# GreenleafLab/NucleoATAC

Measured on AMD Instinct MI355X. Metric: Mbp/s through occ+nuc signal pipeline, higher is better.
Workload: dtype f64

## Files before the change

### nucleoatac_amd/csrc/natac_api.hip

```cpp
#include "../../include/natac.h"
#ifndef NATAC_GNBL
#define NATAC_GNBL 2
#endif
#include "natac_kernels.hpp"
#include "natac_fft_bg.hpp"
#include "natac_occ_fast.hpp"
#include "natac_cand.hpp"
#include "natac_covsweep.hpp"
#include "natac_textz.hpp"
#include "natac_cores.hpp"
#include "natac_writer.hpp"
#include "natac_tabix.hpp"
#include "natac_pack.hpp"
#include "natac_bam.hpp"
#include "natac_bam_dev.hpp"
#include "natac_fragfile.hpp"
#include "natac_fragfile_dev.hpp"
#include "natac_fasta.hpp"
#include "natac_fuzzfit.hpp"
#include "natac_bedtab.hpp"
#include "natac_runtime.hpp"
#include "natac_pwmfit.hpp"
#include "natac_sites.hpp"
#include "natac_cellcounts.hpp"
#include "natac_cellqc.hpp"
#include "natac_peakcall.hpp"
#include "natac_tracks.hpp"
#include "natac_dropins.hpp"
#include "natac_trackio.hpp"
#include "natac_files.hpp"
#include "natac_store.hpp"
#include "natac_profile.hpp"

#include <algorithm>
#include <cmath>
#include <cstdio>
#include <cstring>
#include <limits>
#include <string>
#include <vector>

using namespace natac;

static int need_nuc_geometry(const natac_batch *b, const char *who) {
    const natac_ctx *c = b->ctx;
    const BatchOutputs &o = b->out;
    if (o.nuc_w < 0 || (o.nuc_w == c->vw && o.nuc_lower == c->vlower && o.nuc_upper == c->vupper)) return NATAC_OK;
    return fail(NATAC_E_STATE, "%s: natac_run_nuc ran with the V-plot geometry lower=%d upper=%d w=%d, the context now holds lower=%d "
                "upper=%d w=%d: run natac_run_nuc again", who, o.nuc_lower, o.nuc_upper, o.nuc_w, c->vlower, c->vupper, c->vw);
}
static int need_occ_geometry(const natac_batch *b, const char *who) {
    const natac_ctx *c = b->ctx;
    const BatchOutputs &o = b->out;
    if (o.occ_step < 0 || (o.occ_step == c->step && o.occ_half == c->halfstep && o.occ_flank == c->flank && o.occ_upper == c->occ_upper))
        return NATAC_OK;
    return fail(NATAC_E_STATE, "%s: natac_run_occ ran with step=%d flank=%d upper=%d, the context now holds step=%d flank=%d upper=%d: "
                "run natac_run_occ again", who, o.occ_step, o.occ_flank, o.occ_upper, c->step, c->flank, c->occ_upper);
}

static int choose_bg_G(const natac_batch *b, int W) {
    const int cand[4] = {7, 9, 13, 17};
    double best = 1e300;
    int bestG = 9;
    const int stride = std::max(1, b->nc / 65536);
    for (int ci = 0; ci < 4; ++ci) {
        const int G = cand[ci], TW = 64 * G;
        double cost = 0;
        for (int i = 0; i < b->nc; i += stride) {
            const int nt = (b->h_len[i] + TW - 1) / TW;
            cost += (double)nt * (TW + (W - 1) * 0.15 * 8);
        }
        if (cost < best) { best = cost; bestG = G; }
    }
    return bestG;
}

static void launch_candidates(natac_ctx *c, const ChunkTable &ct, const VMatDev &vm, const int *d_cc, const int *d_cp, long long n,
                              const double *nuc_cov, const double *norm, const double *bnum, const double *bcov, double *lr,
                              double *var, double *z, const long long *tile_first = nullptr, const int2 *ranges256 = nullptr) {
    const int EW = c->W + ((c->vupper - 2) >> 1) + ((c->vupper - 1) >> 1);
    const int ZN = (((c->vupper - 2) >> 1) + ((c->vupper - 1) >> 1) + 5 + 32) & ~1, ON = (c->W + 1) & ~1;
    const size_t lds4 = ((size_t)4 * CAND_PER_WAVE * ((EW + 1) & ~1) + ZN + ON) * sizeof(double);
    const bool per_wave = c->W <= 2 * WAVE;
    const size_t ldsp = (size_t)4 * CAND_PER_WAVE * CANDP_STRIDE * sizeof(double);
    bool paired = per_wave && bnum && bcov && c->vlower >= 2 && (c->R & 1) == 0 && c->W >= 64 && !vm.has_zero && EW <= CANDP_STRIDE &&
                  !getenv("NATAC_CAND_FULL") && !getenv("NATAC_CAND_OLD");
    if (paired && (c->lrt_gen != c->model_gen || !c->d_lrt)) {
        if (c->d_lrt.size() < (size_t)c->R * c->W && dev_alloc(c->d_lrt, (size_t)c->R * c->W) != NATAC_OK)
            paired = false;
        if (paired) {
            hipLaunchKernelGGL(natac_lr_table, dim3((unsigned)((c->R * c->W + 255) / 256)), dim3(256), 0, c->stream, c->d_vmat, c->d_srow, c->R, c->W,
                               c->d_lrt);
            c->lrt_gen = c->model_gen;
        }
    }
    if (paired) {
        VMatDev vml = vm;
        vml.lrt = c->d_lrt;
        const long long per_block = 4 * CAND_PER_WAVE;
        const dim3 grid((unsigned)((n + per_block - 1) / per_block));
        if (c->vlower & 1)
            hipLaunchKernelGGL((natac_candidates_paired<true>), grid, dim3(256), ldsp, c->stream, ct, vml, d_cc, d_cp, (int)n, nuc_cov, norm,
                               bnum, bcov, tile_first, ranges256, lr, var, z);
        else
            hipLaunchKernelGGL((natac_candidates_paired<false>), grid, dim3(256), ldsp, c->stream, ct, vml, d_cc, d_cp, (int)n, nuc_cov, norm,
                               bnum, bcov, tile_first, ranges256, lr, var, z);
        return;
    }
    if (per_wave && lds4 <= 64 * 1024) {
        const long long per_block = 4 * CAND_PER_WAVE;
        if (bnum && bcov && !getenv("NATAC_CAND_FULL"))
            hipLaunchKernelGGL((natac_candidates4<true>), dim3((unsigned)((n + per_block - 1) / per_block)), dim3(256), lds4, c->stream,
                               ct, vm, d_cc, d_cp, (int)n, nuc_cov, norm, bnum, bcov, lr, var, z);
        else
            hipLaunchKernelGGL((natac_candidates4<false>), dim3((unsigned)((n + per_block - 1) / per_block)), dim3(256), lds4, c->stream,
                               ct, vm, d_cc, d_cp, (int)n, nuc_cov, norm, bnum, bcov, lr, var, z);
    } else {
        hipLaunchKernelGGL(natac_candidates, dim3((unsigned)n), dim3(256), (size_t)(EW + 2) * sizeof(double), c->stream, ct, vm, d_cc,
                           d_cp, nuc_cov, norm, lr, var, z);
    }
}

template <int G>
static void launch_bg(natac_batch *b, const ChunkTable &ct, const VMatDev &vm) {
    natac_ctx *c = b->ctx;
    constexpr int W = 121;
    const int PW = 64 * G + W - 1;
    const int EW = PW + ((vm.upper - 2) >> 1) + ((vm.upper - 1) >> 1);
    const size_t lds = ((size_t)((EW + 1) & ~1) + PW) * sizeof(double);
    hipLaunchKernelGGL((natac_background<G, W>), dim3(b->n_tiles_bg), dim3(64), lds, c->stream, ct, b->d_tiles_bg, vm,
                       b->d_track[NATAC_T_NUC_COV], b->d_track[NATAC_T_RAW], b->d_track[NATAC_T_BACKGROUND],
                       b->d_track[NATAC_T_NORM], b->d_bnum, b->d_bcov);
}

struct OccFastLaunch { natac_batch *b; const ChunkTable &ct; const OccFastDev &of; size_t lds_gs, lds_od; int rem; bool rn16; };
template <int STEP, int REM = 0>
static void occ_gsum_launch(const OccFastLaunch &f) {
    if constexpr (REM < STEP) {
        if (f.rem == REM)
            hipLaunchKernelGGL((natac_occ_gsum<STEP, REM>), dim3(f.b->n_tiles_gs), dim3(256), f.lds_gs, f.b->ctx->stream, f.ct, f.b->d_tiles_gs, f.of,
                               f.b->d_blk_off, f.b->total_blocks, f.b->d_gsum);
        else
            occ_gsum_launch<STEP, REM + 1>(f);
    }
}
template <int STEP>
static void occ_fast_launch(const OccFastLaunch &f) {
    natac_batch *b = f.b;
    occ_gsum_launch<STEP>(f);
    auto kd = (f.of.flags & 2) ? (f.rn16 ? natac_occ_decide<STEP, 16, true> : natac_occ_decide<STEP, 4, true>)
                               : (f.rn16 ? natac_occ_decide<STEP, 16, false> : natac_occ_decide<STEP, 4, false>);
    const bool heavy_first = b->ctx->occ_ordered;
    hipLaunchKernelGGL(kd, dim3((b->n_tiles_occ + (heavy_first ? HEAVY_CAP : 0) + 3) / 4), dim3(256), f.lds_od, b->ctx->stream, f.ct, b->d_tiles_occ,
                       b->n_tiles_occ, b->d_ranges_occ, heavy_first ? b->d_order_occ : nullptr, f.of, b->d_blk_off, b->total_blocks, b->d_gsum, b->d_grid[0], b->d_grid[1], b->d_grid[2], b->d_defer,
                       b->d_defer + 1);
}

extern "C" {

int natac_abi_version(void) { return NATAC_ABI_VERSION; }
const char *natac_last_error(void) { return g_err.c_str(); }

int natac_device_count(int *count) {
    if (!count) return fail(NATAC_E_ARG, "count is NULL");
    int n = 0;
    hipError_t e = hipGetDeviceCount(&n);
    if (e != hipSuccess) {
        *count = 0;
        return fail(NATAC_E_HIP, "hipGetDeviceCount: %s", hipGetErrorString(e));
    }
    *count = n;
    return NATAC_OK;
}

int natac_ctx_create(int device_id, natac_ctx **out) {
    if (!out) return fail(NATAC_E_ARG, "out is NULL");
    *out = nullptr;
    int n = 0;
    HIPCHK(hipGetDeviceCount(&n));
    if (device_id < 0 || device_id >= n) return fail(NATAC_E_ARG, "device %d out of range (%d devices)", device_id, n);
    HIPCHK(hipSetDevice(device_id));
// ... 274 lines not shown
    if (rc) return rc;
    HIPCHK(sync_all(b->ctx));
    return NATAC_OK;
}

static int ensure_fft(natac_ctx *c) {
    int rc;
    if (!c->d_fft_tw) {
        std::vector<double> tw(2 * (size_t)natac::FFT_N);
        for (int k = 0; k < natac::FFT_N; ++k) {
            const double a = 2.0 * M_PI * k / natac::FFT_N;
            tw[2 * k] = std::cos(a);
            tw[2 * k + 1] = -std::sin(a);
        }
        if (const char *e = getenv("NATAC_FAULT_TWIDDLE")) {
            int k = 0; double dlt = 0.0;
            if (sscanf(e, "%d:%lf", &k, &dlt) == 2 && k >= 0 && k < natac::FFT_N) tw[2 * (size_t)k] += dlt;
        }
        if ((rc = dev_upload(c, c->d_fft_tw, tw.data(), tw.size()))) return rc;
        HIPCHK(sync_all(c));
    }
    if (!c->fft_dirty) return NATAC_OK;
    HIPCHK(sync_all(c));
    const int npair = (c->R + 1) / 2;
    if ((rc = dev_alloc(c->d_fft_k, (size_t)npair * 2 * natac::FFT_N))) return rc;
    hipLaunchKernelGGL(natac_fft_template, dim3(npair), dim3(64), 0, c->stream, c->d_vmat, c->d_srow, c->R, c->W, c->d_fft_tw, c->d_fft_k);
    if (c->W >= natac::FFT_EXT) {
        c->d_fft_mtab.reset(); c->d_fft_swt.reset();
        const int NJ = (c->R + 3) / 4;
        if ((rc = dev_alloc(c->d_fft_mtab, (size_t)2 * NJ * 64)) || (rc = dev_alloc(c->d_fft_swt, (size_t)4 * NJ))) return rc;
        hipLaunchKernelGGL(natac_fft_edge_table_mfma, dim3((2 * NJ * 64 + 255) / 256), dim3(256), 0, c->stream, c->d_vmat, c->d_srow, c->R, c->W, NJ,
                           c->d_fft_mtab, c->d_fft_swt);
    }
    HIPCHK(hipGetLastError());
    c->fft_dirty = false;
    return NATAC_OK;
}

static int ensure_window(natac_ctx *c, PoolBuf<double> &slot, int *slotM, double *slotsd, int M, double sd, double *slotsum = nullptr) {
    if (slot && *slotM == M && *slotsd == sd) return NATAC_OK;
    HIPCHK(sync_all(c));
    std::vector<double> w((size_t)M);
    for (int i = 0; i < M; ++i) {
        double n = (double)i - (M - 1) / 2.0;
        double q = n / sd;
        w[i] = std::exp(-0.5 * (q * q));
    }
    int rc = dev_upload(c, slot, w.data(), (size_t)M);
    if (rc) return rc;
    HIPCHK(sync_all(c));
    if (slotsum) {
        double acc = 0.0;
        for (int i = 0; i < M; ++i) acc = acc + w[i];
        *slotsum = acc;
    }
    *slotM = M;
    *slotsd = sd;
    return NATAC_OK;
}

static int run_exp_bias(natac_batch *b, hipStream_t st, bool from_occ) {
    if (!b->d_bias) return NATAC_OK;
    if (from_occ && b->ebias_fresh) { b->ebias_fresh = false; return NATAC_OK; }
    b->ebias_fresh = !from_occ;
    int rc;
    if (!b->d_ebias && (rc = dev_alloc(b->d_ebias, (size_t)b->nb))) return rc;
    const int blocks = (int)std::min<long long>((b->nb + 255) / 256, 16384);
    hipLaunchKernelGGL(natac_exp_bias, dim3(blocks), dim3(256), 0, st, b->d_bias, b->d_ebias, b->nb);
    return NATAC_OK;
}

static ChunkTable make_table(natac_batch *b) {
    ChunkTable t;
    t.nc = b->nc; t.chunk_len = b->d_len; t.frag_off = b->d_frag_off; t.lpos = b->d_lpos; t.ilen = b->d_ilen;
    t.centre = b->d_centre; t.bias_off = b->d_bias_off; t.bias = b->d_bias; t.ebias = b->d_ebias; t.bias_left = b->bias_left;
    t.bias_right = b->bias_right; t.out_off = b->d_out_off; t.grid_off = b->d_grid_off;
    return t;
}
static VMatDev make_vmat(natac_ctx *c) {
    VMatDev v;
    v.mat = c->d_vmat; v.matp = c->d_vmat_pad; v.srow = c->d_srow; v.lower = c->vlower; v.upper = c->vupper; v.w = c->vw; v.R = c->R; v.W = c->W;
    v.has_zero = (c->vmat_zero || c->srow_zero) ? 1 : 0;
    v.lrt = nullptr;
    return v;
}
static OccModelDev make_occ(natac_ctx *c) {
    OccModelDev o;
    o.nuc_probs = c->d_nucp; o.nfr_probs = c->d_nfrp; o.alphas = c->d_alphas; o.upper = c->occ_upper;
    o.n_alpha = c->n_alpha; o.step = c->step; o.halfstep = c->halfstep; o.flank = c->flank; o.cutoff = c->cutoff;
    o.ci_factor = std::exp(-0.5 * c->cutoff);
    o.zero_flags = c->occ_zero_flags;
    o.b_floor = c->occ_b_floor;
    return o;
}

static int build_tiles(natac_batch *b, int width, PoolBuf<int2> &d_out, int *n_out, bool grid_units = false, int step = 1, int half = 0) {
    std::vector<int2> tiles;
    tiles.reserve((size_t)(b->total_bp / std::max(1, width)) + b->nc);
    for (int i = 0; i < b->nc; ++i) {
        int n = b->h_len[i];
        if (grid_units) n = (b->h_len[i] > half) ? (b->h_len[i] - half + step - 1) / step : 0;
        for (int x = 0; x < n; x += width) tiles.push_back(make_int2(i, x));
    }
    *n_out = (int)tiles.size();
    int rc = dev_upload(b->ctx, d_out, tiles.data(), tiles.size());
    if (rc) return rc;
    HIPCHK(sync_all(b->ctx));
    return NATAC_OK;
}

int natac_batch_create(natac_ctx *c, int32_t nc, const int32_t *chunk_len, const int64_t *frag_off, const int32_t *frag_lpos,
                       const int32_t *frag_ilen, const int64_t *bias_off, const double *bias_log, int32_t bias_left,
                       int32_t bias_right, natac_batch **out) {
    if (!c || !out || !chunk_len || !frag_off) return fail(NATAC_E_ARG, "null argument");
    *out = nullptr;
    if (nc <= 0) return fail(NATAC_E_ARG, "n_chunks must be positive");
    if (bias_log && !bias_off) return fail(NATAC_E_ARG, "bias_log without bias_off");
    if (frag_off[0] != 0) return fail(NATAC_E_ARG, "frag_off[0] must be 0");
    const long long nf = frag_off[nc];
    if (nf > 0 && (!frag_lpos || !frag_ilen)) return fail(NATAC_E_ARG, "fragment arrays are NULL");
    HIPCHK(hipSetDevice(c->device));
    natac_batch *b = new natac_batch();
    b->ctx = c; b->nc = nc; b->nf = nf; b->bias_left = bias_left; b->bias_right = bias_right;
    b->h_len.assign(chunk_len, chunk_len + nc);
    b->h_out_off.resize((size_t)nc + 1);
    b->h_out_off[0] = 0;
    for (int i = 0; i < nc; ++i) {
        if (chunk_len[i] <= 0) { delete b; return fail(NATAC_E_ARG, "chunk %d has length %d", i, chunk_len[i]); }
        if (frag_off[i + 1] < frag_off[i] || frag_off[i + 1] - frag_off[i] > 0x7fffffffLL) {
            delete b; return fail(NATAC_E_ARG, "frag_off not monotone (chunk %d)", i);
        }
        if (bias_off && bias_off[i + 1] - bias_off[i] != (long long)chunk_len[i] + bias_left + bias_right) {
            delete b; return fail(NATAC_E_ARG, "bias slice of chunk %d must cover [start-%d, end+%d)", i, bias_left, bias_right);
        }
        b->h_out_off[i + 1] = b->h_out_off[i] + chunk_len[i];
    }
    b->total_bp = b->h_out_off[nc];
    b->nb = bias_off ? bias_off[nc] : 0;
    auto upload = [&]() -> int {
        int rc;
        if ((rc = dev_upload(c, b->d_len, chunk_len, (size_t)nc)) ||
            (rc = dev_upload(c, b->d_frag_off, (const long long *)frag_off, (size_t)nc + 1)) ||
            (rc = dev_upload(c, b->d_lpos, frag_lpos, (size_t)nf)) || (rc = dev_upload(c, b->d_ilen, frag_ilen, (size_t)nf)) ||
            (rc = dev_alloc(b->d_centre, (size_t)nf)) || (rc = dev_upload(c, b->d_out_off, b->h_out_off.data(), (size_t)nc + 1)))
            return rc;
        if (bias_off) {
            if ((rc = dev_upload(c, b->d_bias_off, (const long long *)bias_off, (size_t)nc + 1))) return rc;
            if (bias_log) rc = dev_upload(c, b->d_bias, bias_log, (size_t)b->nb);
            else rc = dev_alloc(b->d_bias, (size_t)b->nb);
            if (rc) return rc;
        }
        if ((rc = dev_alloc(b->d_status, (size_t)nc))) return rc;
        hipError_t e = hipMemsetAsync(b->d_status, 0, (size_t)nc * sizeof(int), c->stream);
        if (e != hipSuccess) return fail(NATAC_E_HIP, "memset: %s", hipGetErrorString(e));
        if (nf > 0) {
            int blocks = (int)std::min<long long>((nf + 255) / 256, 4096);
            hipLaunchKernelGGL(natac_frag_centres, dim3(blocks), dim3(256), 0, c->stream, b->d_lpos, b->d_ilen, b->d_centre, nf);
        }
        if ((rc = build_tiles(b, 256, b->d_tiles256, &b->n_tiles256))) return rc;
        {
            std::vector<long long> first((size_t)nc + 1, 0);
            for (int i = 0; i < nc; ++i) first[(size_t)i + 1] = first[i] + (chunk_len[i] + 255) / 256;
            if ((rc = dev_upload(c, b->d_tile256_first, first.data(), first.size()))) return rc;
        }
        e = hipStreamSynchronize(c->stream);
        if (e != hipSuccess) return fail(NATAC_E_HIP, "upload: %s", hipGetErrorString(e));
// ... 1046 lines not shown
```

### nucleoatac_amd/csrc/natac_cand.hpp

```cpp
#pragma once
#include "natac_kernels.hpp"

namespace natac {

__device__ __forceinline__ int row_lower_bound(const int *__restrict__ a, int lo, int hi, int key, int l, int sh) {
    while (__ballot(hi - lo > 16) != 0ull) {
        const int n = hi - lo;
        const bool big = n > 16;
        const int stride = big ? (n + 15) / 16 : 1;
        const int pi = min((l + 1) * stride - 1, max(n - 1, 0));
        const bool less = big && a[lo + pi] < key;
        const int cnt = __popc((unsigned)(__ballot(less) >> sh) & 0xffffu);
        if (big) {
            lo = min(lo + cnt * stride, hi);
            hi = min(lo + stride, hi);
        }
    }
    const int i = lo + l;
    const bool less = (i < hi) && a[i] < key;
    return lo + __popc((unsigned)(__ballot(less) >> sh) & 0xffffu);
}

__global__ void __launch_bounds__(256) natac_lr_table(const double *__restrict__ vmat, const double *__restrict__ srow, int R, int W,
                                                        double *__restrict__ out) {
    const int i = blockIdx.x * 256 + threadIdx.x;
    if (i < R * W) out[i] = log(vmat[i] / srow[i / W]);
}

constexpr int CANDP_STRIDE = 376;

template <bool LODD>
__global__ void __launch_bounds__(256) __attribute__((amdgpu_waves_per_eu(3, 3))) natac_candidates_paired(
    ChunkTable ct, VMatDev vm, const int *__restrict__ cand_chunk, const int *__restrict__ cand_pos, int ncand,
    const double *__restrict__ nuc_cov, const double *__restrict__ norm, const double *__restrict__ bnum,
    const double *__restrict__ bcov, const long long *__restrict__ tile_first, const int2 *__restrict__ ranges256,
    double *__restrict__ out_lr, double *__restrict__ out_var, double *__restrict__ out_z) {
    extern __shared__ __attribute__((aligned(16))) double smem[];
    constexpr int Q = CAND_PER_WAVE;
    const int A = (vm.upper - 2) >> 1, Bh = (vm.upper - 1) >> 1;
    const int W = vm.W, R = vm.R;
    const int EW = W + A + Bh;
    constexpr int EWP = CANDP_STRIDE;
    const int wave = threadIdx.x >> 6, lane = threadIdx.x & 63;
    double *Ew = smem + wave * Q * EWP;
    const int k0 = (blockIdx.x * 4 + wave) * Q;
    if (k0 >= ncand) return;
    int chunk[Q], pos[Q];
    bool esmall = false;
#pragma unroll
    for (int q = 0; q < Q; ++q) {
        const int k = (k0 + q < ncand) ? k0 + q : k0;
        chunk[q] = cand_chunk[k];
        pos[q] = cand_pos[k];
        const int L = ct.chunk_len[chunk[q]];
        const double *b = ct.bias ? ct.ebias + ct.bias_off[chunk[q]] : nullptr;
        const int nb = L + ct.bias_left + ct.bias_right;
        const int j0 = pos[q] - vm.w - A + ct.bias_left;
        double emin = __builtin_inf();
        for (int u = lane; u < EW; u += WAVE) {
            const int j = j0 + u;
            double e = 1.0;
            if (b) e = (j >= 0 && j < nb) ? b[j] : 0.0;
            Ew[q * EWP + u] = e;
            emin = fmin(emin, e);
        }
        esmall |= !(wave_min(emin) > 0x1p-500);
    }
    __builtin_amdgcn_wave_barrier();
    const int c1 = lane, c2 = min(lane + WAVE, W - 1);
    const bool h2 = lane + WAVE < W;
    double a1[Q][2], a2[Q][2];
    double carry[Q][2];
#pragma unroll
    for (int q = 0; q < Q; ++q) { a1[q][0] = a1[q][1] = a2[q][0] = a2[q][1] = 0.0; }
    const int m0 = LODD ? (vm.lower - 1) >> 1 : vm.lower >> 1;
    {
        const int off = LODD ? A + m0 : A - m0 + 1;
#pragma unroll
        for (int q = 0; q < Q; ++q) { carry[q][0] = Ew[q * EWP + c1 + off]; carry[q][1] = Ew[q * EWP + c2 + off]; }
    }
    const double *__restrict__ vmat = vm.mat;
    const int npair = R >> 1;
    const double *psh1 = Ew + c1 + (LODD ? A - m0 : A + m0), *psh2 = Ew + c2 + (LODD ? A - m0 : A + m0);
    const double *pnw1 = Ew + c1 + (LODD ? A + m0 + 1 : A - m0), *pnw2 = Ew + c2 + (LODD ? A + m0 + 1 : A - m0);
    constexpr int DSH = LODD ? -1 : 1, DNW = LODD ? 1 : -1;
    struct PairT { double va0, va1, vb0, vb1, sa, sb; };
    const double hm = h2 ? 1.0 : 0.0;
    const unsigned o1 = (unsigned)c1 * 8u, o2 = (unsigned)c2 * 8u;
    auto load_pair = [&](int k) {
        PairT t;
        t.sa = vm.srow[2 * k]; t.sb = vm.srow[2 * k + 1];
        const char *ra = (const char *)(vmat + (size_t)(2 * k) * (size_t)W), *rb = ra + (size_t)W * sizeof(double);
        t.va0 = *(const double *)(ra + o1); t.va1 = *(const double *)(ra + o2);
        t.vb0 = *(const double *)(rb + o1); t.vb1 = *(const double *)(rb + o2);
        return t;
    };
    auto pair_step = [&](const PairT &t, const double (&cin)[Q][2], double (&cout)[Q][2]) {
        const double va0 = t.va0, va1 = hm * t.va1, vb0 = t.vb0, vb1 = hm * t.vb1;
        const double wa0 = t.sa * (va0 * va0), wa1 = t.sa * (va1 * va1);
        const double wb0 = t.sb * (vb0 * vb0), wb1 = t.sb * (vb1 * vb1);
        double s0[Q], s1[Q];
#pragma unroll
        for (int q = 0; q < Q; ++q) {
            s0[q] = psh1[q * EWP]; s1[q] = psh2[q * EWP];
            cout[q][0] = pnw1[q * EWP]; cout[q][1] = pnw2[q * EWP];
        }
        __builtin_amdgcn_sched_barrier(0);
#pragma unroll
        for (int q = 0; q < Q; ++q) {
            const double n0 = cout[q][0], n1 = cout[q][1];
            a1[q][0] = fma(s0[q], fma(vb0, n0, va0 * cin[q][0]), a1[q][0]);
            a1[q][1] = fma(s1[q], fma(vb1, n1, va1 * cin[q][1]), a1[q][1]);
            a2[q][0] = fma(s0[q], fma(wb0, n0, wa0 * cin[q][0]), a2[q][0]);
            a2[q][1] = fma(s1[q], fma(wb1, n1, wa1 * cin[q][1]), a2[q][1]);
        }
        psh1 += DSH; psh2 += DSH; pnw1 += DNW; pnw2 += DNW;
    };
    double carry2[Q][2];
    int k = 0;
    PairT t0 = load_pair(0), t1 = load_pair(min(1, npair - 1));
    for (; k + 4 <= npair; k += 4) {
        const PairT u0 = load_pair(min(k + 2, npair - 1));
        pair_step(t0, carry, carry2);
        const PairT u1 = load_pair(min(k + 3, npair - 1));
        pair_step(t1, carry2, carry);
        t0 = load_pair(min(k + 4, npair - 1));
        pair_step(u0, carry, carry2);
        t1 = load_pair(min(k + 5, npair - 1));
        pair_step(u1, carry2, carry);
    }
    for (; k + 2 <= npair; k += 2) {
        const PairT u0 = load_pair(min(k + 2, npair - 1));
        pair_step(t0, carry, carry2);
        t0 = u0;
        const PairT u1 = load_pair(min(k + 3, npair - 1));
        pair_step(t1, carry2, carry);
        t1 = u1;
    }
    if (k < npair) pair_step(t0, carry, carry2);
    bool zero[Q];
#pragma unroll
    for (int q = 0; q < Q; ++q) zero[q] = false;
    if (esmall) {
        for (int r = 0; r < R; ++r) {
            const int i = vm.lower + r;
            const int hl = floor_half(i - 1), hr = floor_half(i);
            const double sr = vm.srow[r];
            const double v1 = vmat[r * W + c1], v2 = vmat[r * W + c2];
#pragma unroll
            for (int q = 0; q < Q; ++q) {
                const double *e = Ew + q * EWP;
                const double b1 = e[c1 + A - hl] * e[c1 + A + hr], b2 = e[c2 + A - hl] * e[c2 + A + hr];
                zero[q] |= (v1 * b1 == 0.0 || sr * b1 == 0.0) || (h2 && (v2 * b2 == 0.0 || sr * b2 == 0.0));
            }
        }
    }
    double tBV2[Q], tB0V[Q];
    bool anyzero[Q];
#pragma unroll
    for (int q = 0; q < Q; ++q) {
        tB0V[q] = wave_sum(a1[q][0] + a1[q][1]);
        tBV2[q] = wave_sum(a2[q][0] + a2[q][1]);
        anyzero[q] = __ballot(zero[q]) != 0ull;
    }
    const int row = lane >> 4, l = lane & 15, sh = 16 * row;
    int mych = chunk[0], myp = pos[0];
    double myB0V = tB0V[0], myBV2 = tBV2[0];
    bool myzero = anyzero[0];
#pragma unroll
    for (int q = 1; q < Q; ++q)
        if (row == q) { mych = chunk[q]; myp = pos[q]; myB0V = tB0V[q]; myBV2 = tBV2[q]; myzero = anyzero[q]; }
    const long long op = ct.out_off[mych] + myp;
    const double tB = bcov[op], tBV = bnum[op];
    const int nfr = (int)(ct.frag_off[mych + 1] - ct.frag_off[mych]);
    const int *cen = ct.centre + ct.frag_off[mych];
    const int *iln = ct.ilen + ct.frag_off[mych];
    int f0, f1;
    if (ranges256) {
        const int2 tr = ranges256[tile_first[mych] + (myp >> 8)];
        const int klo = myp - vm.w, khi = myp + vm.w + 1;
        int below_lo = 0, below_hi = 0;
        int span = tr.y - tr.x;
        span = max(max(__builtin_amdgcn_readlane(span, 0), __builtin_amdgcn_readlane(span, 16)),
                   max(__builtin_amdgcn_readlane(span, 32), __builtin_amdgcn_readlane(span, 48)));
        for (int base = 0; base < span; base += 64) {
            int cv[4];
#pragma unroll
            for (int it = 0; it < 4; ++it) {
                const int i = tr.x + base + 16 * it + l;
                cv[it] = 0x7fffffff;
                if (i < tr.y) cv[it] = cen[i];
            }
#pragma unroll
            for (int it = 0; it < 4; ++it) {
                below_lo += __popc((unsigned)(__ballot(cv[it] < klo) >> sh) & 0xffffu);
                below_hi += __popc((unsigned)(__ballot(cv[it] < khi) >> sh) & 0xffffu);
            }
        }
        f0 = tr.x + below_lo;
        f1 = tr.x + below_hi;
    } else {
        f0 = row_lower_bound(cen, 0, nfr, myp - vm.w, l, sh);
        f1 = row_lower_bound(cen, f0, nfr, myp + vm.w + 1, l, sh);
    }
    const double *__restrict__ lrt = vm.lrt;
    double acc = 0.0, cntf = 0.0;
    int fmax = f1 - f0;
    fmax = max(max(__builtin_amdgcn_readlane(fmax, 0), __builtin_amdgcn_readlane(fmax, 16)),
               max(__builtin_amdgcn_readlane(fmax, 32), __builtin_amdgcn_readlane(fmax, 48)));
    {
        int nn[4], cc[4];
#pragma unroll
        for (int it = 0; it < 4; ++it) {
            const int f = f0 + 16 * it + l;
            nn[it] = -1; cc[it] = 0;
            if (f < f1) { nn[it] = iln[f]; cc[it] = cen[f]; }
        }
        double tv[4];
#pragma unroll
        for (int it = 0; it < 4; ++it) {
            tv[it] = 0.0;
            if (nn[it] >= vm.lower && nn[it] < vm.upper) tv[it] = lrt[(nn[it] - vm.lower) * W + (cc[it] - myp + vm.w)];
// ... 26 lines not shown
```

### nucleoatac_amd/csrc/natac_kernels.hpp

```cpp
#pragma once
#include <hip/hip_runtime.h>
#include <stdint.h>

#include <type_traits>

namespace natac {

constexpr int WAVE = 64;

struct ChunkTable {
    int nc;
    const int *chunk_len;
    const long long *frag_off;
    const int *lpos;
    const int *ilen;
    const int *centre;
    const long long *bias_off;
    const double *bias;
    const double *ebias;
    int bias_left, bias_right;
    const long long *out_off;
    const long long *grid_off;
};

constexpr int VPAD = 128;

struct VMatDev {
    const double *mat;
    const double *matp;
    const double *srow;
    const double *lrt;
    int lower, upper, w, R, W;
    int has_zero;
};

__device__ __forceinline__ int floor_half(int x) { return x >> 1; }

__host__ __device__ __forceinline__ double cov_reads(double x) {
    if (x != x) return x;
    const double t = x < 0 ? ceil(x) : floor(x);
    if (t == 0.0) return 0.0;
    return t < -2147483648.0 ? -2147483648.0 : (t > 2147483647.0 ? 2147483647.0 : t);
}

__device__ __forceinline__ int lower_bound_i32(const int *a, int lo, int hi, int key) {
    while (lo < hi) {
        int mid = (lo + hi) >> 1;
        if (a[mid] < key) lo = mid + 1; else hi = mid;
    }
    return lo;
}

template <int CTRL>
__device__ __forceinline__ double dpp_mov_f64(double v) {
    const int lo = __builtin_amdgcn_update_dpp(0, __double2loint(v), CTRL, 0xf, 0xf, false);
    const int hi = __builtin_amdgcn_update_dpp(0, __double2hiint(v), CTRL, 0xf, 0xf, false);
    return __hiloint2double(hi, lo);
}
__device__ __forceinline__ double readlane_f64(double v, int lane) {
    const int lo = __builtin_amdgcn_readlane(__double2loint(v), lane);
    const int hi = __builtin_amdgcn_readlane(__double2hiint(v), lane);
    return __hiloint2double(hi, lo);
}
__device__ __forceinline__ double wave_sum(double v) {
    v += dpp_mov_f64<0xB1>(v);
    v += dpp_mov_f64<0x4E>(v);
    v += dpp_mov_f64<0x141>(v);
    v += dpp_mov_f64<0x140>(v);
    return (readlane_f64(v, 0) + readlane_f64(v, 16)) + (readlane_f64(v, 32) + readlane_f64(v, 48));
}
__device__ __forceinline__ double wave_min(double v) {
    v = fmin(v, dpp_mov_f64<0xB1>(v));
    v = fmin(v, dpp_mov_f64<0x4E>(v));
    v = fmin(v, dpp_mov_f64<0x141>(v));
    v = fmin(v, dpp_mov_f64<0x140>(v));
    return fmin(fmin(readlane_f64(v, 0), readlane_f64(v, 16)), fmin(readlane_f64(v, 32), readlane_f64(v, 48)));
}
__device__ __forceinline__ double wave_max(double v) {
    v = fmax(v, dpp_mov_f64<0xB1>(v));
    v = fmax(v, dpp_mov_f64<0x4E>(v));
    v = fmax(v, dpp_mov_f64<0x141>(v));
    v = fmax(v, dpp_mov_f64<0x140>(v));
    return fmax(fmax(readlane_f64(v, 0), readlane_f64(v, 16)), fmax(readlane_f64(v, 32), readlane_f64(v, 48)));
}
__device__ __forceinline__ int wave_or(int v) {
    int r = 0;
#pragma unroll
    for (int bit = 1; bit <= 8; bit <<= 1)
        if (__ballot((v & bit) != 0) != 0ull) r |= bit;
    return r;
}
__device__ __forceinline__ double row_sum(double v) {
    v += dpp_mov_f64<0xB1>(v);
    v += dpp_mov_f64<0x4E>(v);
    v += dpp_mov_f64<0x141>(v);
    v += dpp_mov_f64<0x140>(v);
    return v;
}
__device__ __forceinline__ double row_max(double v) {
    v = fmax(v, dpp_mov_f64<0xB1>(v));
    v = fmax(v, dpp_mov_f64<0x4E>(v));
    v = fmax(v, dpp_mov_f64<0x141>(v));
    v = fmax(v, dpp_mov_f64<0x140>(v));
    return v;
}
template <int CTRL>
__device__ __forceinline__ int dpp_mov_i32(int v) { return __builtin_amdgcn_update_dpp(0, v, CTRL, 0xf, 0xf, false); }
__device__ __forceinline__ int row_min_i32(int v) {
    v = min(v, dpp_mov_i32<0xB1>(v));
    v = min(v, dpp_mov_i32<0x4E>(v));
    v = min(v, dpp_mov_i32<0x141>(v));
    v = min(v, dpp_mov_i32<0x140>(v));
    return v;
}
// ... 2126 lines not shown
```

### nucleoatac_amd/csrc/natac_runtime.hpp

```cpp
#pragma once
#include "../../include/natac.h"
#include "natac_textz.hpp"

#include <algorithm>
#include <cstdarg>
#include <cstdio>
#include <cstdlib>
#include <map>
#include <mutex>
#include <string>
#include <unordered_map>
#include <utility>
#include <vector>

static thread_local std::string g_err;

static int fail(int code, const char *fmt, ...) {
    char buf[512];
    va_list ap;
    va_start(ap, fmt);
    vsnprintf(buf, sizeof buf, fmt, ap);
    va_end(ap);
    g_err = buf;
    return code;
}

#define HIPCHK(expr)                                                                                  \
    do {                                                                                              \
        hipError_t e_ = (expr);                                                                       \
        if (e_ != hipSuccess)                                                                         \
            return fail(e_ == hipErrorOutOfMemory ? NATAC_E_NOMEM : NATAC_E_HIP, "%s: %s (%s:%d)", #expr, \
                        hipGetErrorString(e_), __FILE__, __LINE__);                                   \
    } while (0)

static hipError_t pool_alloc(void **p, size_t bytes);
static void dev_free(void *p);

template <class T>
class PoolBuf {
  public:
    PoolBuf() = default;
    PoolBuf(PoolBuf &&o) noexcept : p_(o.p_), n_(o.n_) { o.p_ = nullptr; o.n_ = 0; }
    PoolBuf &operator=(PoolBuf &&o) noexcept {
        if (this != &o) { reset(); p_ = o.p_; n_ = o.n_; o.p_ = nullptr; o.n_ = 0; }
        return *this;
    }
    ~PoolBuf() { reset(); }
    void reset() { dev_free(p_); p_ = nullptr; n_ = 0; }
    hipError_t alloc(size_t n) {
        reset();
        if (n == 0) n = 1;
        void *p = nullptr;
        const hipError_t e = pool_alloc(&p, n * sizeof(T));
        if (e == hipSuccess) { p_ = (T *)p; n_ = n; }
        return e;
    }
    T *get() const { return p_; }
    operator T *() const { return p_; }
    size_t size() const { return n_; }

  private:
    T *p_ = nullptr;
    size_t n_ = 0;
};

template <class T>
static int dev_alloc(PoolBuf<T> &buf, size_t n) {
    HIPCHK(buf.alloc(n));
    return NATAC_OK;
}

struct natac_ctx {
    int device = 0;
    hipStream_t stream = nullptr;
    hipStream_t copy_stream = nullptr;
    hipDeviceProp_t prop;
    PoolBuf<double> d_vmat, d_vmat_pad, d_srow, d_sizes;
    PoolBuf<double> d_lrt;
    long long lrt_gen = -1;
    int vlower = 0, vupper = 0, vw = 0, R = 0, W = 0, sizes_upper = 0;
    bool have_vmat = false, have_sizes = false, srow_dirty = true;
    bool vmat_zero = false, srow_zero = false;
    long long model_gen = 0;
    PoolBuf<double> d_fft_tw, d_fft_k;
    PoolBuf<double> d_fft_mtab, d_fft_swt;
    bool bg_ext = true;
    bool fft_dirty = true, bg_direct = false, occ_ordered = true, occ_zero_nfr = false;
    std::vector<double> h_sizes;
    PoolBuf<double> d_nucp, d_nfrp, d_alphas;
    int occ_upper = 0, n_alpha = 0, step = 0, halfstep = 0, flank = 0;
    double cutoff = 0;
    bool have_occ = false;
    int occ_zero_flags = 0;
    PoolBuf<double> d_occ_q4, d_occ_rho;
    int occ_nm = 0;
    bool occ_fast_ok = false, occ_force_general = false, occ_rn16 = false;
    double occ_b_floor = 0;
    PoolBuf<double> d_win_nuc, d_win_occ;
    PoolBuf<double> d_wb_occ;
    int wb_M = 0, wb_step = 0;
    int win_nuc_M = 0, win_occ_M = 0;
    double win_nuc_sd = -1, win_occ_sd = -1;
    double win_nuc_sum = 0, win_occ_sum = 0;
    bool profiling = false;
    struct Ev { int k; hipEvent_t a, b; hipStream_t st; };
    std::vector<Ev> pending;
    double prof_ms[NATAC_K_COUNT] = {0};
    int64_t prof_n[NATAC_K_COUNT] = {0};
    hipEvent_t t0 = nullptr, t1 = nullptr;
    hipStream_t ck_stream = nullptr;
    hipEvent_t ck_start = nullptr;
    long long *d_ck = nullptr;
    int ck_cap = 0;
    bool ck_active = false;
    struct Iv { int k; float t0, t1; };
    std::vector<Iv> ck_iv;
    PoolBuf<natac_text::P10> d_p10;
    PoolBuf<natac_deflate::CrcTables> d_crc;
};

enum TrackState : unsigned char { TS_EMPTY = 0, TS_PENDING, TS_RUN , TS_HOST  };
struct BatchOutputs {
    TrackState track[NATAC_T_COUNT] = {};
    bool grids = false;
    long long bg_gen = -1;
    int nuc_w = -1, nuc_lower = -1, nuc_upper = -1;
    bool occ_cov_by_nuc = false;
    int occ_step = -1, occ_half = -1, occ_flank = -1, occ_upper = -1;
};

struct natac_batch {
    natac_ctx *ctx = nullptr;
    int nc = 0;
    long long nf = 0, nb = 0, total_bp = 0, total_grid = 0;
    int bias_left = 0, bias_right = 0;
    std::vector<int> h_len;
    std::vector<long long> h_out_off, h_grid_off;
    PoolBuf<int> d_len, d_lpos, d_ilen, d_centre, d_status;
    PoolBuf<long long> d_frag_off, d_bias_off, d_out_off, d_grid_off;
    PoolBuf<double> d_bias, d_ebias;
    PoolBuf<unsigned long long> d_occ_minkey;
    PoolBuf<int> d_occ_nan;
    int n_tiles_os = 0, os_width = 0;
    PoolBuf<int2> d_tiles_os, d_tiles1k;
    int n_tiles1k = 0;
    PoolBuf<int2> d_tiles256, d_tiles_bg, d_tiles_occ, d_ranges_occ, d_ranges256;
    PoolBuf<long long> d_tile256_first;
    PoolBuf<int> d_order_occ;
    int ranges256_w = -1;
    int ranges_occ_key[3] = {-1, -1, -1};
    int n_tiles256 = 0, n_tiles_bg = 0, n_tiles_occ = 0, bgG = 0;
    int grid_step = 0, grid_half = 0;
    PoolBuf<long long> d_blk_off;
    long long total_blocks = 0;
    PoolBuf<double> d_gsum;
    PoolBuf<int2> d_tiles_gs;
    int n_tiles_gs = 0, gs_Q = -1;
    PoolBuf<int> d_defer;
    PoolBuf<double> d_opk_vals, d_nuc_dist;
    PoolBuf<int> d_opk_keep;
    long long opk_cap = 0, opk_n = -1;
    int nd_upper = 0;
// ... 242 lines not shown
```

Baseline: 3604.

## Repack vmat row pairs into a lane-interleaved table for vectorized candidate loads

Adds a cached device table, rebuilt whenever the model generation changes, that stores each pair of vmat rows in a lane-interleaved layout. Each lane's two columns sit side by side, so the paired candidate kernel reads them with one 16-byte load addressed by an immediate offset from a single running pointer. The LDS reads in the inner loop also switch to integer indices with compile-time offsets, and the h2 mask multiply is dropped because the table zero-pads columns beyond W. The aim is to cut address arithmetic and memory instructions in the hot pair loop, at the cost of an extra table buffer and a one-time build kernel.

Result: faster. 3655, median of 6 (+1.4%).

```diff
diff --git a/nucleoatac_amd/csrc/natac_api.hip b/nucleoatac_amd/csrc/natac_api.hip
--- a/nucleoatac_amd/csrc/natac_api.hip
+++ b/nucleoatac_amd/csrc/natac_api.hip
@@ -94,9 +94,18 @@
             c->lrt_gen = c->model_gen;
         }
     }
+    if (paired && (c->ctab_gen != c->model_gen || !c->d_ctab)) {
+        const size_t nd = cand_table_doubles(c->R);
+        if (c->d_ctab.size() < nd && dev_alloc(c->d_ctab, nd) != NATAC_OK) paired = false;
+        if (paired) {
+            hipLaunchKernelGGL(natac_cand_table, dim3((unsigned)((nd / 2 + 255) / 256)), dim3(256), 0, c->stream, c->d_vmat, c->R, c->W, c->d_ctab);
+            c->ctab_gen = c->model_gen;
+        }
+    }
     if (paired) {
         VMatDev vml = vm;
         vml.lrt = c->d_lrt;
+        vml.ctab = c->d_ctab;
         const long long per_block = 4 * CAND_PER_WAVE;
         const dim3 grid((unsigned)((n + per_block - 1) / per_block));
         if (c->vlower & 1)
@@ -537,6 +546,7 @@
     v.mat = c->d_vmat; v.matp = c->d_vmat_pad; v.srow = c->d_srow; v.lower = c->vlower; v.upper = c->vupper; v.w = c->vw; v.R = c->R; v.W = c->W;
     v.has_zero = (c->vmat_zero || c->srow_zero) ? 1 : 0;
     v.lrt = nullptr;
+    v.ctab = nullptr;
     return v;
 }
 static OccModelDev make_occ(natac_ctx *c) {
diff --git a/nucleoatac_amd/csrc/natac_cand.hpp b/nucleoatac_amd/csrc/natac_cand.hpp
--- a/nucleoatac_amd/csrc/natac_cand.hpp
+++ b/nucleoatac_amd/csrc/natac_cand.hpp
@@ -25,6 +25,23 @@
                                                         double *__restrict__ out) {
     const int i = blockIdx.x * 256 + threadIdx.x;
     if (i < R * W) out[i] = log(vmat[i] / srow[i / W]);
+}
+
+constexpr int CAND_TAB_PAD = 2;
+constexpr int CAND_TAB_PAIR = WAVE * 4;
+__host__ __device__ constexpr size_t cand_table_doubles(int R) { return (size_t)((R >> 1) + CAND_TAB_PAD) * CAND_TAB_PAIR; }
+__global__ void __launch_bounds__(256) natac_cand_table(const double *__restrict__ vmat, int R, int W, double *__restrict__ out) {
+    const int i = blockIdx.x * 256 + threadIdx.x;
+    const int k = i >> 7, row = (i >> 6) & 1, l = i & 63;
+    if (k >= (R >> 1) + CAND_TAB_PAD) return;
+    double v0 = 0.0, v1 = 0.0;
+    if (k < (R >> 1)) {
+        const double *r = vmat + (size_t)(2 * k + row) * W;
+        v0 = r[l];
+        if (l + WAVE < W) v1 = r[l + WAVE];
+    }
+    out[(size_t)i * 2] = v0;
+    out[(size_t)i * 2 + 1] = v1;
 }
 
 constexpr int CANDP_STRIDE = 376;
@@ -81,29 +98,31 @@
     }
     const double *__restrict__ vmat = vm.mat;
     const int npair = R >> 1;
-    const double *psh1 = Ew + c1 + (LODD ? A - m0 : A + m0), *psh2 = Ew + c2 + (LODD ? A - m0 : A + m0);
-    const double *pnw1 = Ew + c1 + (LODD ? A + m0 + 1 : A - m0), *pnw2 = Ew + c2 + (LODD ? A + m0 + 1 : A - m0);
     constexpr int DSH = LODD ? -1 : 1, DNW = LODD ? 1 : -1;
+    constexpr int BSH = DSH < 0 ? 3 : 0, BNW = DNW < 0 ? 3 : 0;
+    const int ew0 = wave * Q * EWP;
+    int ish1 = ew0 + c1 + (LODD ? A - m0 : A + m0) - BSH, ish2 = ew0 + c2 + (LODD ? A - m0 : A + m0) - BSH;
+    int inw1 = ew0 + c1 + (LODD ? A + m0 + 1 : A - m0) - BNW, inw2 = ew0 + c2 + (LODD ? A + m0 + 1 : A - m0) - BNW;
+    asm("" : "+v"(ish1), "+v"(ish2), "+v"(inw1), "+v"(inw2));
     struct PairT { double va0, va1, vb0, vb1, sa, sb; };
-    const double hm = h2 ? 1.0 : 0.0;
-    const unsigned o1 = (unsigned)c1 * 8u, o2 = (unsigned)c2 * 8u;
-    auto load_pair = [&](int k) {
-        PairT t;
-        t.sa = vm.srow[2 * k]; t.sb = vm.srow[2 * k + 1];
-        const char *ra = (const char *)(vmat + (size_t)(2 * k) * (size_t)W), *rb = ra + (size_t)W * sizeof(double);
-        t.va0 = *(const double *)(ra + o1); t.va1 = *(const double *)(ra + o2);
-        t.vb0 = *(const double *)(rb + o1); t.vb1 = *(const double *)(rb + o2);
-        return t;
+    constexpr int PAIRB = CAND_TAB_PAIR * (int)sizeof(double);
+    const char *ctab = (const char *)vm.ctab;
+    unsigned vo = (unsigned)lane * 16u + 4u * PAIRB;
+    asm("" : "+v"(vo));
+    auto load_pair = [&](int kk, int imm) {
+        const double2 *p = (const double2 *)(ctab + (size_t)vo + (ptrdiff_t)imm);
+        const double2 a = p[0], b = p[WAVE];
+        return PairT{a.x, a.y, b.x, b.y, vm.srow[2 * kk], vm.srow[2 * kk + 1]};
     };
-    auto pair_step = [&](const PairT &t, const double (&cin)[Q][2], double (&cout)[Q][2]) {
-        const double va0 = t.va0, va1 = hm * t.va1, vb0 = t.vb0, vb1 = hm * t.vb1;
+    auto pair_step = [&](const PairT &t, const double (&cin)[Q][2], double (&cout)[Q][2], auto osh, auto onw) {
+        const double va0 = t.va0, va1 = t.va1, vb0 = t.vb0, vb1 = t.vb1;
         const double wa0 = t.sa * (va0 * va0), wa1 = t.sa * (va1 * va1);
         const double wb0 = t.sb * (vb0 * vb0), wb1 = t.sb * (vb1 * vb1);
         double s0[Q], s1[Q];
 #pragma unroll
         for (int q = 0; q < Q; ++q) {
-            s0[q] = psh1[q * EWP]; s1[q] = psh2[q * EWP];
-            cout[q][0] = pnw1[q * EWP]; cout[q][1] = pnw2[q * EWP];
+            s0[q] = smem[ish1 + (q * EWP + osh)]; s1[q] = smem[ish2 + (q * EWP + osh)];
+            cout[q][0] = smem[inw1 + (q * EWP + onw)]; cout[q][1] = smem[inw2 + (q * EWP + onw)];
         }
         __builtin_amdgcn_sched_barrier(0);
 #pragma unroll
@@ -114,30 +133,34 @@
             a2[q][0] = fma(s0[q], fma(wb0, n0, wa0 * cin[q][0]), a2[q][0]);
             a2[q][1] = fma(s1[q], fma(wb1, n1, wa1 * cin[q][1]), a2[q][1]);
         }
-        psh1 += DSH; psh2 += DSH; pnw1 += DNW; pnw2 += DNW;
     };
+#define NATAC_OFF(J, B, D) std::integral_constant<int, (B) + (J) * (D)>{}
     double carry2[Q][2];
     int k = 0;
-    PairT t0 = load_pair(0), t1 = load_pair(min(1, npair - 1));
+    PairT t0 = load_pair(0, -4 * PAIRB), t1 = load_pair(min(1, npair - 1), -3 * PAIRB);
     for (; k + 4 <= npair; k += 4) {
-        const PairT u0 = load_pair(min(k + 2, npair - 1));
-        pair_step(t0, carry, carry2);
-        const PairT u1 = load_pair(min(k + 3, npair - 1));
-        pair_step(t1, carry2, carry);
-        t0 = load_pair(min(k + 4, npair - 1));
-        pair_step(u0, carry, carry2);
-        t1 = load_pair(min(k + 5, npair - 1));
-        pair_step(u1, carry2, carry);
-    }
+        const PairT u0 = load_pair(min(k + 2, npair - 1), -2 * PAIRB);
+        pair_step(t0, carry, carry2, NATAC_OFF(0, BSH, DSH), NATAC_OFF(0, BNW, DNW));
+        const PairT u1 = load_pair(min(k + 3, npair - 1), -PAIRB);
+        pair_step(t1, carry2, carry, NATAC_OFF(1, BSH, DSH), NATAC_OFF(1, BNW, DNW));
+        t0 = load_pair(min(k + 4, npair - 1), 0);
+        pair_step(u0, carry, carry2, NATAC_OFF(2, BSH, DSH), NATAC_OFF(2, BNW, DNW));
+        t1 = load_pair(min(k + 5, npair - 1), PAIRB);
+        pair_step(u1, carry2, carry, NATAC_OFF(3, BSH, DSH), NATAC_OFF(3, BNW, DNW));
+        ish1 += 4 * DSH; ish2 += 4 * DSH; inw1 += 4 * DNW; inw2 += 4 * DNW;
+        vo += 4u * PAIRB;
+    }
+    ish1 += BSH; ish2 += BSH; inw1 += BNW; inw2 += BNW;
     for (; k + 2 <= npair; k += 2) {
-        const PairT u0 = load_pair(min(k + 2, npair - 1));
-        pair_step(t0, carry, carry2);
-        t0 = u0;
-        const PairT u1 = load_pair(min(k + 3, npair - 1));
-        pair_step(t1, carry2, carry);
-        t1 = u1;
-    }
-    if (k < npair) pair_step(t0, carry, carry2);
+        pair_step(t0, carry, carry2, NATAC_OFF(0, 0, DSH), NATAC_OFF(0, 0, DNW));
+        t0 = load_pair(min(k + 2, npair - 1), -2 * PAIRB);
+        pair_step(t1, carry2, carry, NATAC_OFF(1, 0, DSH), NATAC_OFF(1, 0, DNW));
+        t1 = load_pair(min(k + 3, npair - 1), -PAIRB);
+        ish1 += 2 * DSH; ish2 += 2 * DSH; inw1 += 2 * DNW; inw2 += 2 * DNW;
+        vo += 2u * PAIRB;
+    }
+    if (k < npair) pair_step(t0, carry, carry2, NATAC_OFF(0, 0, DSH), NATAC_OFF(0, 0, DNW));
+#undef NATAC_OFF
     bool zero[Q];
 #pragma unroll
     for (int q = 0; q < Q; ++q) zero[q] = false;
diff --git a/nucleoatac_amd/csrc/natac_kernels.hpp b/nucleoatac_amd/csrc/natac_kernels.hpp
--- a/nucleoatac_amd/csrc/natac_kernels.hpp
+++ b/nucleoatac_amd/csrc/natac_kernels.hpp
@@ -30,6 +30,7 @@
     const double *matp;
     const double *srow;
     const double *lrt;
+    const double *ctab;
     int lower, upper, w, R, W;
     int has_zero;
 };
diff --git a/nucleoatac_amd/csrc/natac_runtime.hpp b/nucleoatac_amd/csrc/natac_runtime.hpp
--- a/nucleoatac_amd/csrc/natac_runtime.hpp
+++ b/nucleoatac_amd/csrc/natac_runtime.hpp
@@ -78,6 +78,8 @@
     PoolBuf<double> d_vmat, d_vmat_pad, d_srow, d_sizes;
     PoolBuf<double> d_lrt;
     long long lrt_gen = -1;
+    PoolBuf<double> d_ctab;
+    long long ctab_gen = -1;
     int vlower = 0, vupper = 0, vw = 0, R = 0, W = 0, sizes_upper = 0;
     bool have_vmat = false, have_sizes = false, srow_dirty = true;
     bool vmat_zero = false, srow_zero = false;
diff --git a/profiles/r7_cand_table/count_isa.py b/profiles/r7_cand_table/count_isa.py
--- /dev/null
+++ b/profiles/r7_cand_table/count_isa.py
@@ -0,0 +1,72 @@
+#!/usr/bin/env python3
+import re
+import sys
+from collections import Counter, OrderedDict
+
+
+def classify(op):
+    if op.startswith("v_"):
+        return "valu"
+    if op.startswith("ds_"):
+        return "lds"
+    if op.startswith(("global_", "flat_", "buffer_", "scratch_")):
+        return "vmem"
+    if op.startswith(("s_load", "s_buffer_load")):
+        return "smem"
+    if op.startswith("s_waitcnt"):
+        return "wait"
+    if op.startswith(("s_cbranch", "s_branch")):
+        return "branch"
+    if op.startswith("s_"):
+        return "salu"
+    return "other"
+
+
+def main():
+    path, key = sys.argv[1], sys.argv[2]
+    lines = open(path).read().split("\n")
+    start = next(i for i, l in enumerate(lines) if key in l and l.rstrip().split(";")[0].rstrip().endswith(":") and not l.startswith("\t"))
+    end = next(i for i in range(start, len(lines)) if lines[i].startswith("\t.amdhsa_kernel") or ".Lfunc_end" in lines[i] and lines[i].endswith(":"))
+    blocks = OrderedDict()
+    cur = "entry"
+    blocks[cur] = []
+    for l in lines[start + 1:end]:
+        s = l.split(";")[0].strip()
+        if not s or s.startswith("."):
+            m = re.match(r"^(\.LBB\d+_\d+):", s)
+            if m:
+                cur = m.group(1)
+                blocks[cur] = []
+            continue
+        blocks[cur].append(s)
+    for l in lines[end:]:
+        if re.search(r"; (NumVgprs|NumAgprs|ScratchSize|Occupancy|SGPRBlocks|NumSgprs|LDSByteSize|codeLenInByte)", l):
+            print(l.strip())
+        if l.startswith("\t.section") and ".text" in l and key not in l:
+            break
+    order = list(blocks)
+    total = Counter()
+    print("%-12s %6s %6s %6s %6s %6s %6s %6s  %s" % ("block", "valu", "lds", "vmem", "smem", "salu", "wait", "all", "notes"))
+    for name, ins in blocks.items():
+        c = Counter(classify(i.split()[0]) for i in ins)
+        ops = Counter(i.split()[0] for i in ins)
+        total.update(c)
+        note = ""
+        for i in ins:
+            m = re.match(r"s_cbranch\S*\s+(\.LBB\d+_\d+)|s_branch\s+(\.LBB\d+_\d+)", i)
+            if m:
+                tgt = m.group(1) or m.group(2)
+                if tgt in order and order.index(tgt) <= order.index(name):
+                    note += " loop->" + tgt
+        f64 = sum(v for k, v in ops.items() if k in ("v_fma_f64", "v_mul_f64", "v_add_f64", "v_pk_fma_f64"))
+        if f64:
+            note += " fp64=%d" % f64
+        print("%-12s %6d %6d %6d %6d %6d %6d %6d %s" % (name, c["valu"], c["lds"], c["vmem"], c["smem"], c["salu"], c["wait"], len(ins), note))
+        if "-v" in sys.argv and "loop->" in note:
+            for k, v in sorted(ops.items(), key=lambda kv: -kv[1]):
+                print("      %-28s %d" % (k, v))
+    print("%-12s %6d %6d %6d %6d %6d %6d %6d" % ("total", total["valu"], total["lds"], total["vmem"], total["smem"], total["salu"], total["wait"], sum(total.values())))
+
+
+if __name__ == "__main__":
+    main()
```
